# raahii/dcvgan

Measured on AMD Instinct MI355X. Metric: videos/sec per G+D step, 16x64x64 RGB+depth, higher is better.
Workload: dtype f32

## Files before the change

### dcvgan_amd/csrc/conv_mfma.hip

```cpp
#include "dcv_common.h"

#include <algorithm>
#include <cstdlib>
#include <map>
#include <mutex>
#include <string>
#include <type_traits>
#include <vector>

namespace dcv {

thread_local char g_err[512] = {0};
std::atomic<uint64_t> g_launches{0};
thread_local char g_last_kernel[160] = {0};
#define DCV_NOTE_KERNEL(...) snprintf(g_last_kernel, sizeof(g_last_kernel), __VA_ARGS__)

typedef float f32x16 __attribute__((ext_vector_type(16)));
typedef __bf16 bf16x8 __attribute__((ext_vector_type(8)));

std::atomic<int> g_precision{0};
struct BnView {
    const float* bx; const float* gamma; const float* beta; const float* mean; const float* invstd;
    int64_t bx_sn;
    int32_t bx_sc, bx_sh, cbn, act;
// ... 817 lines not shown
#else
#define DCV_STAMP_OUT()
#endif

    if (slabmode) {
        float* __restrict__ sl = a.slab + (int64_t)blockIdx.y * a.OCp * a.slab_mp;
#pragma unroll
        for (int j = 0; j < TM; ++j)
#pragma unroll
            for (int i = 0; i < TOC; ++i)
#pragma unroll
                for (int r = 0; r < 16; ++r) {
                    const int oc = oc0 + (woc * TOC + i) * 32 + (r & 3) + 8 * (r >> 2) + 4 * lhi;
                    sl[(int64_t)oc * a.slab_mp + (m0 - a.rag_m0) + (wm * TM + j) * 32 + l31] = acc[i][j][r];
                }
        DCV_STAMP_OUT()
        return;
    }
    gather_epilogue<TOC, TM>(a, acc, m0, wm * TM * 32, l31, lhi, oc0 + woc * TOC * 32, n0);
    if (a.stat) tile_bn_partials<TOC, TM, WOC, WM>(a, acc, smem, tid, lane, woc, wm, oc0, m_t);
    DCV_STAMP_OUT()
}

__global__ __launch_bounds__(256) void splitk_reduce_kernel(const GatherArgsPack pack, int S) {
    const GatherArgs& a = pack.c[blockIdx.y];
    const uint32_t Mp = (uint32_t)a.slab_mp, M = (uint32_t)a.M, q4 = Mp >> 2;
    if (q4 == 0) return;
    const uint32_t idx = blockIdx.x * 256u + threadIdx.x;
    const uint32_t oc = idx / q4, ml = (idx - oc * q4) * 4, m = ml + (uint32_t)a.rag_m0;
    if (oc >= (uint32_t)a.OC || m >= M) return;
    const float4* __restrict__ p = reinterpret_cast<const float4*>(a.slab + (int64_t)oc * Mp + ml);
    const int64_t stride = ((int64_t)a.OCp * Mp) >> 2;
    float4 v0 = {0.f, 0.f, 0.f, 0.f}, v1 = v0, v2 = v0, v3 = v0;
    int k = 0;
    for (; k + 3 < S; k += 4) {
        const float4 t0 = p[(int64_t)k * stride], t1 = p[(int64_t)(k + 1) * stride], t2 = p[(int64_t)(k + 2) * stride], t3 = p[(int64_t)(k + 3) * stride];
        v0.x += t0.x; v0.y += t0.y; v0.z += t0.z; v0.w += t0.w;
        v1.x += t1.x; v1.y += t1.y; v1.z += t1.z; v1.w += t1.w;
        v2.x += t2.x; v2.y += t2.y; v2.z += t2.z; v2.w += t2.w;
        v3.x += t3.x; v3.y += t3.y; v3.z += t3.z; v3.w += t3.w;
    }
    for (; k < S; ++k) {
        const float4 t0 = p[(int64_t)k * stride];
        v0.x += t0.x; v0.y += t0.y; v0.z += t0.z; v0.w += t0.w;
    }
    const float v[4] = {(v0.x + v1.x) + (v2.x + v3.x), (v0.y + v1.y) + (v2.y + v3.y), (v0.z + v1.z) + (v2.z + v3.z), (v0.w + v1.w) + (v2.w + v3.w)};
    const int act = a.act, accumulate = a.accumulate;
    const float slope = a.slope;
    float* __restrict__ yb = a.y + a.y_off + (int64_t)oc * a.y_sc;
#pragma unroll
    for (int e = 0; e < 4; ++e) {
        const uint32_t me = m + e;
        if (me >= M) break;
        const uint32_t n = fdiv(me, a.div_sp);
        uint32_t r0 = me - n * a.div_sp.div;
        const uint32_t od = fdiv(r0, a.div_hw);
        r0 -= od * a.div_hw.div;
        const uint32_t oh = fdiv(r0, a.div_w);
        const uint32_t ow = r0 - oh * a.div_w.div;
        float* q = yb + (int64_t)n * a.y_sn + (int64_t)od * a.y_sd + (int64_t)oh * a.y_sh + (int64_t)ow * a.y_sw;
        float x = v[e];
        if (accumulate) x += *q;
        if (a.gate) x *= a.gate[q - a.y] > 0.f ? 1.f : a.gate_slope;
        *q = apply_act(x, act, slope);
    }
}

__global__ __launch_bounds__(256) void thin_gather_kernel(const GatherArgs a) {
    __shared__ float red[3][4][64];
    const int tid = threadIdx.x, lane = tid & 63;
    const int wave = __builtin_amdgcn_readfirstlane(tid >> 6);
    const int m0 = blockIdx.x * 64;
    const uint32_t n0 = fdiv((uint32_t)m0, a.div_sp);
    const __amdgpu_buffer_rsrc_t xrs = __builtin_amdgcn_make_buffer_rsrc(
        const_cast<float*>(a.x + (int64_t)n0 * a.x_sn), 0, 0x80000000u, 0x00020000);
    const int m = m0 + lane;
    int xbase4 = 0;
    uint32_t vmask = 0;
    uint32_t n = 0, od = 0, oh = 0, ow = 0;
    if (m < a.M) {
        n = fdiv((uint32_t)m, a.div_sp);
        uint32_t r = (uint32_t)m - n * a.div_sp.div;
        od = fdiv(r, a.div_hw);
        r -= od * a.div_hw.div;
        oh = fdiv(r, a.div_w);
        ow = r - oh * a.div_w.div;
        vmask = dim_mask(a.td, (int)od, 0) | dim_mask(a.th, (int)oh, 8) | dim_mask(a.tw, (int)ow, 16);
// ... 2053 lines not shown
        else if (pt) hipLaunchKernelGGL((gather_gemm_dma_kernel<A, B, C_, D, false, true, BF_>), grid, dim3(256), 0, stream, pend); \
        else hipLaunchKernelGGL((gather_gemm_dma_kernel<A, B, C_, D, false, false, BF_>), grid, dim3(256), 0, stream, pend);        \
    }
#define DCV_LAUNCH_DMA(A, B, C_, D)                                                                                           \
    {                                                                                                                         \
        if (bfm == 2) DCV_LAUNCH_DMA1(A, B, C_, D, 2) else if (bfm == 1) DCV_LAUNCH_DMA1(A, B, C_, D, 1) else DCV_LAUNCH_DMA1(A, B, C_, D, 0) \
    }
    if (tc.bn == 128 && tc.bm == 64) DCV_LAUNCH_DMA(2, 1, 2, 2)
    else if (tc.bn == 64 && tc.bm == 128) DCV_LAUNCH_DMA(2, 1, 1, 4)
    else if (tc.bn == 128) DCV_LAUNCH_DMA(2, 2, 2, 2)
    else if (tc.bn == 64) DCV_LAUNCH_DMA(2, 2, 1, 4)
    else DCV_LAUNCH_DMA(1, 2, 1, 4)
#undef DCV_LAUNCH_DMA
#undef DCV_LAUNCH_DMA1
    DCV_NOTE_KERNEL("gather_gemm_dma_kernel<%s, %s, %s, %s> (%d x %d tile, %d class%s in one launch%s%s)",
                    tc.bn == 128 ? (tc.bm == 64 ? "2, 1, 2, 2" : "2, 2, 2, 2") : tc.bn == 64 ? (tc.bm == 128 ? "2, 1, 1, 4" : "2, 2, 1, 4") : "1, 2, 1, 4",
                    ds ? "true" : "false", pt ? "true" : "false", bfm == 2 ? "2" : bfm ? "1" : "0", tc.bn, tc.bm, n, n == 1 ? "" : "es", KS > 1 ? (pend.c[0].rag_m0 > 0 ? ", ragged split-K" : ", split-K") : "",
                    bfm == 2 ? ", f32x6: fp32 on the bf16 pipe" : bfm ? ", bf16 products" : "");
    DCV_LAUNCH_CHECK();
    if (KS > 1) {
        int64_t tot = 0;
        for (int i = 0; i < n; ++i) tot = std::max<int64_t>(tot, (int64_t)OC * (pend.c[i].slab_mp / 4));
        if (tot == 0) return DCV_OK;
        hipLaunchKernelGGL(splitk_reduce_kernel, dim3((unsigned)((tot + 255) / 256), (unsigned)n), dim3(256), 0, stream, pend, KS);
        DCV_LAUNCH_CHECK();
    }
    return DCV_OK;
}

static int structured_walk(const GatherClass& c, const dcv_dims5& xd, int RC, bool dstep, bool thin) {
    if (thin) return 0;
    if (dstep) return 2;
    const int nd = c.taps[0].n, THW = c.taps[1].n * c.taps[2].n, T = nd * THW;
    const int64_t sc4 = xd.sc * 4;
    if (T > 0 && 16 % T == 0 && RC % (16 / T) == 0 && sc4 * (16 / T) < (1ll << 30)) return 1;
    if (THW == 16 && (nd == 2 || nd == 4 || nd == 8) && c.taps[0].mul == 1 && c.taps[0].base == 0 &&
        c.taps[0].delta[nd - 1] == nd - 1 && c.o_ext[0] + nd - 1 <= c.taps[0].size && sc4 < (1ll << 30)) return 3;
    return 0;
}

static inline size_t pack_elem_bytes(int precision) { return precision == 2 ? 6 : sizeof(float); }

struct GatherOp {
    const float* x = nullptr; float* y = nullptr; const float* w = nullptr;
    dcv_dims5 xd{}, yd{};
    int RC = 0, OC = 0, KH = 1, KW = 1;
    int64_t ws_o = 0, ws_r = 0;
// ... 35 lines not shown
    const int RC = op.RC, OC = op.OC;
    const char* tag = op.tag;
    TileCfg tc = pick_gather_tile(OC);
    int nlive = 0, stat_ntm = 0, ntm_min = INT32_MAX;
    auto workgroups = [&](int bm) {
        int64_t W = 0;
        for (const GatherClass& c : op.classes)
            if (live(c)) W += ((OC + tc.bn - 1) / tc.bn) * (((int64_t)yd.n * c.o_ext[0] * c.o_ext[1] * c.o_ext[2] + bm - 1) / bm);
        return W;
    };
    for (const GatherClass& c : op.classes) nlive += live(c);
    if (tc.bn >= 64) {
        const int64_t W = workgroups(tc.bm);
        const double rounds = (double)W / 1024.0, frac = rounds - (double)(int64_t)rounds;
        bool half = (rounds > 0.4 && rounds < 1.0) || (rounds >= 1.0 && rounds < 3.0 && frac > 0.15 && frac < 0.55);
        if (tg.half_m >= 0) half = tg.half_m != 0;
        if (half && rounds >= 1.0 && tg.half_m < 0 && !tg.no_lds_dma && nlive > 0 && W / nlive >= 384 &&
            rag_plan(W, ((OC + tc.bn - 1) / tc.bn) * nlive).k > 1) half = false;
        if (half) tc.bm /= 2;
    }
    RagPlan rag{0, 1};
    if (tc.bn >= 64 && !tg.no_lds_dma) {
        rag = rag_plan(workgroups(tc.bm), ((OC + tc.bn - 1) / tc.bn) * nlive);
        if (op.stats && (int64_t)OC * yd.n * yd.d * yd.h * yd.w * 4 > (160ll << 20)) rag.k = 1;
    }
    if (op.gate && tc.bn == 4) return fail(DCV_EUNSUPPORTED, "%s: the gated epilogue is not built into the thin (OC <= 4) kernels", tag);
    if (op.gate)
        for (const GatherClass& c : op.classes)
            if (c.taps[0].n * c.taps[1].n * c.taps[2].n == 0 && c.o_ext[0] > 0 && c.o_ext[1] > 0 && c.o_ext[2] > 0)
                return fail(DCV_EUNSUPPORTED, "%s: gated epilogue with a tap-less position class", tag);
    const int OCp = (OC + tc.bn - 1) / tc.bn * tc.bn;
    P->tc = tc; P->OCp = OCp; P->cls.clear(); P->pack_need = 0;
    for (const GatherClass& c : op.classes) {
        if (!live(c)) continue;
        const int ntm = (int)(((int64_t)yd.n * c.o_ext[0] * c.o_ext[1] * c.o_ext[2] + tc.bm - 1) / tc.bm);
        stat_ntm = std::max(stat_ntm, ntm);
        ntm_min = std::min(ntm_min, ntm);
    }
    P->stat_need = (size_t)nlive * stat_ntm * OCp * 2 * sizeof(float);
    bool stat_ok = op.stats && op.act == DCV_ACT_NONE && !op.accumulate && tc.bn != 4 && P->stat_need > 0 && P->stat_need <= op.stat_bytes;
    P->stat_memset = stat_ok && ntm_min != stat_ntm;
    const bool own_pack = op.pack && op.pack->buf;
    size_t pk_off = 0, ws_off = 0;
    int stat_ci = 0;
    for (size_t ci = 0; ci < op.classes.size(); ++ci) {
        const GatherClass& c = op.classes[ci];
        if (!live(c)) continue;
// ... 53 lines not shown
        cp.fmt = dma ? o.precision : 0;
        cp.dstep = dstep; cp.T = T; cp.KS2 = KS2;
        GatherArgs& a = cp.a;
        a.M = (int)M64; a.OC = OC; a.OCp = OCp; a.KIT = KIT;
        a.OD = c.o_ext[0]; a.OH = c.o_ext[1]; a.OW = c.o_ext[2];
        a.div_sp = make_fastdiv((uint32_t)(c.o_ext[0] * c.o_ext[1] * c.o_ext[2]));
        a.div_hw = make_fastdiv((uint32_t)(c.o_ext[1] * c.o_ext[2]));
        a.div_w = make_fastdiv((uint32_t)c.o_ext[2]);
        a.td = c.taps[0]; a.th = c.taps[1]; a.tw = c.taps[2];
        {
            const int64_t per = (int64_t)c.o_ext[0] * c.o_ext[1] * c.o_ext[2];
            const int64_t span = (tc.bm / per + 2) * (xd.sn < 0 ? -xd.sn : xd.sn) + (int64_t)RC * (xd.sc < 0 ? -xd.sc : xd.sc);
            if (span >= (1ll << 29) || xd.sd > INT32_MAX / 256 || xd.sh > INT32_MAX / 256 || xd.sw > INT32_MAX / 256)
                return fail(DCV_EUNSUPPORTED, "%s: input too large for 32-bit block offsets", tag);
            const int64_t yspan = (tc.bm / per + 2) * yd.sn + (int64_t)yd.d * yd.sd + (int64_t)yd.h * yd.sh + (int64_t)yd.w * yd.sw + 8 * yd.sc;
            if (yd.sn < 0 || yd.sc < 0 || yd.sd < 0 || yd.sh < 0 || yd.sw < 0 || yspan >= (1ll << 29) || (int64_t)OCp * yd.sc >= (1ll << 30))
                return fail(DCV_EUNSUPPORTED, "%s: output too large for 32-bit block offsets", tag);
        }
        a.x_sn = xd.sn; a.x_sd = (int32_t)xd.sd; a.x_sh = (int32_t)xd.sh; a.x_sw = (int32_t)xd.sw;
        a.y_sn = yd.sn; a.y_sc = yd.sc; a.y_sd = yd.sd * c.out_mul[0]; a.y_sh = yd.sh * c.out_mul[1]; a.y_sw = yd.sw * c.out_mul[2];
        a.y_off = yd.sd * c.out_off[0] + yd.sh * c.out_off[1] + yd.sw * c.out_off[2];
        a.act = op.act; a.slope = op.slope; a.accumulate = op.accumulate; a.gate_slope = op.gate_slope;
        a.kper = kper; a.Mp = Mp; a.slab_mp = slab_mp; a.rag_m0 = rag_m0;
        cp.stat = stat_ok && KS2 == 1;
        a.stat_ntm = stat_ntm; a.stat_cls = stat_ci++;
        bool thin_struct = false;
        if (tc.bn == 4 && (T == 4 || T == 9 || T == 16) && xd.sc * 4 < (1ll << 30) && (KS2 == 1 || (kper * 16) % T == 0)) {
            thin_struct = true;
            const int nh = c.taps[1].n, nw = c.taps[2].n, THW = nh * nw;
            a.s_stepA = (int32_t)(xd.sc * 4);
            for (int t = 0; t < T; ++t) {
                const int ud = t / THW, uh = (t / nw) % nh, uw = t % nw;
                a.s_local[t] = (int32_t)(4 * (c.taps[0].delta[ud] * xd.sd + c.taps[1].delta[uh] * xd.sh + c.taps[2].delta[uw] * xd.sw));
                a.s_sel[t] = (1u << ud) | (1u << (8 + uh)) | (1u << (16 + uw));
            }
        }
        {
            const int nd = c.taps[0].n, nh = c.taps[1].n, nw = c.taps[2].n, THW = nh * nw;
            const int64_t sc4 = xd.sc * 4;
            a.structured = 0;
            if (walk == 2) {
                a.structured = 2;
                a.s_log2p = nd == 2 ? 1 : nd == 4 ? 2 : 3;
                a.s_stepA = (int32_t)(sc4 * 4);
                a.s_stepD = (int32_t)(4 * xd.sd);
                a.x_back = (int32_t)((nd - 1) * xd.sd);
                for (int r = 0; r < 16; ++r) {
// ... 35 lines not shown
            const bool contig = tap_span(c.taps[1], &dminh) && tap_span(c.taps[2], &dminw);
            const int dw1 = nw >= 2 ? c.taps[2].delta[1] - c.taps[2].delta[0] : 0;
            const bool pairs = (nw == 2 || nw == 4) && (dw1 == 1 || dw1 == -1) && (nw == 2 || c.taps[2].delta[3] - c.taps[2].delta[2] == dw1);
            const int iwmin = c.taps[2].base + dminw;
            const int IWp = IW + 8, GPR = IW / 4 + 2;
            const int l2nh = ilog2(nh), l2ow = ilog2(OW);
            const bool aligned = xd.sw == 1 && IW % 4 == 0 && xd.sh % 4 == 0 && xd.sc % 4 == 0 && xd.sd % 4 == 0 && xd.sn % 4 == 0 &&
                                 (reinterpret_cast<uintptr_t>(op.x) & 15) == 0 && (a.structured != 2 || a.x_back % 4 == 0);
            if (CH > 0 && CH * nh * nw == 16 && contig && pairs && l2nh >= 0 && l2ow >= 0 && OW <= tc.bm && aligned && iwmin >= -4 &&
                (OW - 1) * c.taps[2].mul + iwmin + nw - 1 <= IW + 3 && xd.sc * 4 * CH < (1ll << 30)) {
                const int TR = tc.bm / OW;
                const int G = CH * TR * nh * GPR;
                if (G <= 4 * tc.bm) {
                    a.patch = 1; a.p_G = G; a.p_log2nh = l2nh; a.p_log2tr = ilog2(TR); a.p_log2ow = l2ow; a.p_iwp = IWp;
                    a.p_ihmin = c.taps[1].base + dminh; a.p_iwmin4 = iwmin + 4; a.p_dw1 = dw1; a.p_sc4 = (int32_t)(xd.sc * 4);
                    a.p_gpr = make_fastdiv((uint32_t)GPR);
                    for (int r = 0; r < 16; ++r) {
                        const int t = r % (nh * nw), chr = r / (nh * nw), uh = t / nw, uw = t % nw;
                        a.s_local[r] = 4 * (chr * (TR * nh * IWp) + (c.taps[1].delta[uh] - dminh) * IWp + (c.taps[2].delta[uw] - dminw));
                    }
                }
            }
        }
        if (!dma || KS2 > 1) stat_ok = false;
        if (dma) {
            cp.kind = GK::Dma;
            cp.grid = dim3((unsigned)blocks, (unsigned)KS2);
#ifdef DCV_DEBUG_TIMING
            if (tg.debug_nostore) a.p_pad2 = 0x5701;
#endif
            P->cls.push_back(cp);
            continue;
        }
        int rows_kind = 0;
        if (tc.bn == 4 && KS2 == 1 && xd.sw == 1 && c.taps[0].mul == 1 && c.taps[1].mul == 1 && c.taps[2].mul == 1 &&
            c.o_ext[2] == c.taps[2].size && !tg.no_row64 && xd.sc * 4 < (1ll << 30) && xd.sd * 4 * 8 < (1ll << 30)) {
            const int nd = c.taps[0].n, nh = c.taps[1].n, nw = c.taps[2].n, OWc = c.o_ext[2], OHc = c.o_ext[1];
            if (nd == 1 && nh == 3 && nw == 3 && OWc == 64 && OHc % 4 == 0) rows_kind = 1;
            else if (nd == 1 && nh == 2 && nw == 2 && OWc == 32 && OHc % 8 == 0) rows_kind = 2;
            else if (nd == 4 && nh == 2 && nw == 2 && OWc == 32 && OHc % 8 == 0) rows_kind = 3;
            if (rows_kind) {
                int dminh = 0, dminw = 0;
                const bool ok = tap_span(c.taps[1], &dminh) && tap_span(c.taps[2], &dminw);
                cp.rows_iw0 = c.taps[2].base + dminw;
                if (!ok || cp.rows_iw0 < -1 || cp.rows_iw0 + nw - 1 > 1 || (rows_kind == 1 && cp.rows_iw0 != -1)) rows_kind = 0;
                else {
                    a.p_ihmin = c.taps[1].base + dminh;
// ... 41 lines not shown
                    cp.groups = OHc % 16 == 0 ? 4 : OHc % 8 == 0 ? 2 : 1;
                    cp.grid = dim3((unsigned)(M64 / 256 / cp.groups));
                    cp.kind = GK::WidenMfma;
                    if (const HeadBnRequest* hb = o.headbn) {
                        if (OCp == 128 && OC == 128 && (hb->cbn == 32 || hb->cbn == 64 || hb->cbn == 96) && !op.accumulate && op.act == DCV_ACT_NONE && c.o_ext[0] == 1 &&
                            hb->bxd.n == yd.n && hb->bxd.c == hb->cbn && hb->bxd.d == 1 && hb->bxd.h == OHc && hb->bxd.w == 64 &&
                            hb->bxd.sn >= 0 && hb->bxd.sc >= 0 && hb->bxd.sh >= 0 && hb->bxd.sw >= 0 &&
                            (int64_t)hb->cbn * hb->bxd.sc + (int64_t)OHc * hb->bxd.sh + 64 * hb->bxd.sw < (1ll << 29) &&
                            (size_t)cp.grid.x * hb->cbn * 2 * sizeof(float) <= hb->partial_bytes &&
                            hb->bdxd.sn >= 0 && hb->bdxd.sc >= 0 && hb->bdxd.sh >= 0 && hb->bdxd.sw >= 0 &&
                            (int64_t)hb->cbn * hb->bdxd.sc + (int64_t)OHc * hb->bdxd.sh + 64 * hb->bdxd.sw < (1ll << 29))
                            cp.kind = GK::HeadBn;
                    }
                }
                P->cls.push_back(cp);
                continue;
            }
        }
        cp.kind = tc.bn != 4 ? GK::Gemm : thin_struct ? GK::ThinStruct : GK::ThinGather;
        cp.grid = dim3((unsigned)blocks, (unsigned)KS2);
        P->cls.push_back(cp);
    }
    P->ws_need = ws_off;
    P->stat_parts = stat_ok ? nlive * stat_ntm : 0;
    return DCV_OK;
}

static int gather_table(const GatherOp& op, const ClassPlan& cp, DevTable* tab) {
    const GatherClass& c = op.classes[cp.ci];
    const dcv_dims5& xd = op.xd;
    std::string key = device_prefix() + op.tag;
    {
        char buf[512];
        int nn = snprintf(buf, sizeof(buf), "|g%d|%d|%d|%lld|%lld|%d|%d|%lld|%lld|%lld|%lld|", (int)cp.dstep, op.RC, op.OC, (long long)op.ws_o, (long long)op.ws_r, op.KH, op.KW,
                          (long long)xd.sc, (long long)xd.sd, (long long)xd.sh, (long long)xd.sw);
        key.append(buf, nn);
        for (int d = 0; d < 3; ++d) {
            nn = snprintf(buf, sizeof(buf), "%d:", c.taps[d].n);
            key.append(buf, nn);
            for (int u = 0; u < c.taps[d].n; ++u) {
                nn = snprintf(buf, sizeof(buf), "%d,%d;", c.taps[d].delta[u], c.tap_k[d][u]);
                key.append(buf, nn);
            }
        }
    }
    return get_table(key, [&] {
// ... 69 lines not shown
        }
        break;
    }
    default: {
        const int KS2 = cp.KS2, T = cp.T;
        DCV_NOTE_KERNEL("%s (%d x %d tile%s)", cp.kind == GK::ThinStruct ? "thin_struct_kernel" : cp.kind == GK::ThinGather ? "thin_gather_kernel" : "gather_gemm_kernel",
                        tc.bn, tc.bm, KS2 > 1 ? ", split-K" : "");
        if (cp.kind == GK::ThinStruct) {
            const int rcps = KS2 > 1 ? a.kper * 16 / T : RC;
            if (T == 4) launch_thin_struct<4>(a, OC, RC, rcps, cp.grid, stream);
            else if (T == 9) launch_thin_struct<9>(a, OC, RC, rcps, cp.grid, stream);
            else launch_thin_struct<16>(a, OC, RC, rcps, cp.grid, stream);
        } else if (cp.kind == GK::ThinGather) hipLaunchKernelGGL(thin_gather_kernel, cp.grid, dim3(256), 0, stream, a);
        else if (tc.bn == 128 && tc.bm == 64) launch_gather<2, 1, 2, 2>(a, cp.grid, stream);
        else if (tc.bn == 64 && tc.bm == 128) launch_gather<2, 1, 1, 4>(a, cp.grid, stream);
        else if (tc.bn == 128) launch_gather<2, 2, 2, 2>(a, cp.grid, stream);
        else if (tc.bn == 64) launch_gather<2, 2, 1, 4>(a, cp.grid, stream);
        else launch_gather<1, 2, 1, 4>(a, cp.grid, stream);
        DCV_LAUNCH_CHECK();
        if (KS2 == 1) return DCV_OK;
        const int64_t tot = (int64_t)OC * (a.Mp / 4);
        GatherArgsPack one;
        for (int i = 0; i < 4; ++i) one.c[i] = a;
        hipLaunchKernelGGL(splitk_reduce_kernel, dim3((unsigned)((tot + 255) / 256), 1), dim3(256), 0, stream, one, KS2);
        break;
    }
    }
    DCV_LAUNCH_CHECK();
    return DCV_OK;
}

static int run_gather(const GatherOp& op, const GatherPlan& P, const CallOpts& o, const dcv_wpack* pack, void* ws, hipStream_t stream) {
    const TileCfg& tc = P.tc;
    const bool own_pack = pack && pack->buf;
    char* const wp_base = static_cast<char*>(own_pack ? pack->buf : ws);
    const bool pk_ready = own_pack && pack->ready;
    if (P.stat_memset) DCV_HIP_CHECK(hipMemsetAsync(op.stat, 0, P.stat_need, stream));
    GatherArgsPack pend;
    PackArgs packs;
    memset(&packs, 0, sizeof(packs));
    int npack = 0, packmax = 0, npend = 0, KSpend = 1;
    dim3 pend_grid(0, 1, 1);
    auto flush_pk = [&]() {
        if (npack == 0) return (int)DCV_OK;
        const int rc = flush_packs(op.w, packs, npack, packmax, op.OC, P.OCp, op.ws_o, stream);
        npack = packmax = 0;
        return rc;
// ... 792 lines not shown
    if (pack && pack->buf) { pk2 = *pack; pk2.ready = 1; c.pack = &pk2; }
    if ((rc = run_conv(c, P, o, ws, ws_bytes, stream)) != DCV_OK) return rc;
    *fused = 1;
    return DCV_OK;
}

size_t dcv_conv_packed_bytes(const dcv_conv_geom* g, const dcv_dims5* x, const dcv_dims5* y, int which) {
    ConvPlan P;
    return (which == 0 || which == 1) && plan_sizes(g, x, y, which, false, &P) == DCV_OK ? P.gp.pack_need : 0;
}

int dcv_conv_forward(const dcv_conv_geom* g, const float* x, const dcv_dims5* xd, const float* w, float* y, const dcv_dims5* yd,
                     int act, float slope, const dcv_wpack* pack, void* ws, size_t ws_bytes, void* stream) {
    ConvCall c;
    c.g = g; c.xd = xd; c.yd = yd; c.src = x; c.w = w; c.dst = y; c.act = act; c.slope = slope; c.pack = pack;
    return conv_call(c, ws, ws_bytes, stream);
}

size_t dcv_conv_stats_bytes(const dcv_conv_geom* g, const dcv_dims5* x, const dcv_dims5* y) {
    ConvPlan P;
    return plan_sizes(g, x, y, 0, true, &P) == DCV_OK && P.op.stats ? P.gp.stat_need : 0;
}

int dcv_conv_forward_stats(const dcv_conv_geom* g, const float* x, const dcv_dims5* xd, const float* w, float* y, const dcv_dims5* yd,
                           float* stat, size_t stat_bytes, int* nparts, int* pitch, const dcv_wpack* pack, void* ws, size_t ws_bytes, void* stream) {
    if (!stat || !nparts || !pitch) return fail(DCV_EINVAL, "conv_forward_stats: null pointer");
    CallOpts o; ConvCall c; ConvPlan P;
    int rc = call_opts(g, &o, "conv");
    if (rc != DCV_OK) return rc;
    c.g = g; c.xd = xd; c.yd = yd; c.src = x; c.w = w; c.dst = y; c.pack = pack;
    c.stats = true; c.stat = stat; c.stat_bytes = stat_bytes;
    if ((rc = plan_conv(c, o, &P)) != DCV_OK) return rc;
    *pitch = P.gp.OCp;
    return run_conv(c, P, o, ws, ws_bytes, stream, nparts);
}

int dcv_conv_backward_data(const dcv_conv_geom* g, const float* dy, const dcv_dims5* dyd, const float* w, float* dx, const dcv_dims5* dxd,
                           int accumulate, const dcv_wpack* pack, void* ws, size_t ws_bytes, void* stream) {
    ConvCall c;
    c.which = 1; c.g = g; c.xd = dxd; c.yd = dyd; c.src = dy; c.w = w; c.dst = dx; c.accumulate = accumulate; c.pack = pack;
    return conv_call(c, ws, ws_bytes, stream);
}

int dcv_conv_backward_data_gated(const dcv_conv_geom* g, const float* dy, const dcv_dims5* dyd, const float* w, float* dx, const dcv_dims5* dxd,
                                 int accumulate, const float* x, const dcv_dims5* xd, int act, float slope, const dcv_wpack* pack,
                                 void* ws, size_t ws_bytes, void* stream) {
// ... 72 lines not shown
```

### dcvgan_amd/layers.py

```python
from __future__ import annotations

import torch
import torch.nn as nn

from . import ops, ops_cl

import os

_FUSE_BN_STATS = os.environ.get("DCV_NO_BN_FUSION") is None
KINK_TAP = None
PREBN_TAP = None


def _tap(y, fused):
    if KINK_TAP is not None and fused is not None and fused[0] == ops.ACT_LEAKY:
        KINK_TAP.append((y.detach() > 0).cpu())
_CONVS = (nn.Conv2d, nn.Conv3d, nn.ConvTranspose2d)
_BNS = (nn.BatchNorm2d, nn.BatchNorm3d)


def _act_of(layer):
    if isinstance(layer, nn.LeakyReLU):
        return ops.ACT_LEAKY, float(layer.negative_slope)
    if isinstance(layer, nn.ReLU):
# ... 36 lines not shown
        layer = layers[i]
        nxt = layers[i + 1] if i + 1 < n else None
        if isinstance(layer, _CONVS) and ops_cl.is_cl(x):
            fused = _act_of(nxt) if nxt is not None else None
            last = i + (2 if fused is not None else 1) >= n
            box = [] if (fused is None and isinstance(nxt, _BNS) and nxt.training and _FUSE_BN_STATS) else None
            x = ops_cl.conv(x, layer.weight, geom_of(layer), *(fused or (ops.ACT_NONE, 0.0)), out=out if last else None, grad_slot=grad_slot if i == 0 else None, bn_stats=box,
                            act_slot=act_slot if (last and fused is not None) else None)
            pending = box[0] if box else None
            if PREBN_TAP is not None and fused is None and isinstance(nxt, _BNS):
                PREBN_TAP.append(x.detach().float().abs().max())
            i += 2 if fused is not None else 1
        elif isinstance(layer, _CONVS):
            fused = _act_of(nxt) if nxt is not None else None
            if fused is not None:
                x = ops.conv(x, layer.weight, geom_of(layer), fused[0], fused[1], out=out if i + 2 >= n else None, grad_slot=grad_slot if i == 0 else None,
                             act_slot=act_slot if i + 2 >= n else None, bn_link=bn_link if i == 0 else None, gate=gate if first_conv else None)
                first_conv = False
                _tap(x, fused)
                i += 2
            else:
                box = [] if (isinstance(nxt, _BNS) and nxt.training and _FUSE_BN_STATS) else None
                x = ops.conv(x, layer.weight, geom_of(layer), out=out if i + 1 >= n else None, bn_stats=box, grad_slot=grad_slot if i == 0 else None,
                             gate=gate if first_conv else None)
                first_conv = False
                pending = box[0] if box else None
                i += 1
        elif isinstance(layer, _BNS):
            j = i + 1
            drop = None
            if j < n and isinstance(layers[j], nn.Dropout2d):
                drop = layers[j]
                j += 1
            fused = _act_of(layers[j]) if j < n else None
            if fused is not None:
                j += 1
            x = batch_norm(layer, x, rng, fused or (ops.ACT_NONE, 0.0), drop, out=out if j >= n else None, partials=pending,
                           link=bn_link if (j >= n and not ops_cl.is_cl(x)) else None)
            _tap(x, fused)
            pending = None
            i = j
        elif _act_of(layer) is not None:
            code, slope = _act_of(layer)
            x = ops_cl.act(x, code, slope) if ops_cl.is_cl(x) else ops.act(x, code, slope)
            _tap(x, (code, slope))
            i += 1
        elif hasattr(layer, "use_noise") and hasattr(layer, "sigma"):
# ... 14 lines not shown
```

### dcvgan_amd/native.py

```python
from __future__ import annotations

import ctypes as C
import os
import threading
from typing import Optional, Sequence

import torch

_HERE = os.path.dirname(os.path.abspath(__file__))
LIB_PATH = os.environ.get("DCV_LIB_PATH") or os.path.join(_HERE, "libdcvgan_hip.so")

ACT_NONE, ACT_LEAKY, ACT_TANH = 0, 1, 2
DCV_OK, DCV_EINVAL, DCV_EWORKSPACE, DCV_EHIP, DCV_EUNSUPPORTED = 0, -1, -2, -3, -4


class NativeError(RuntimeError):
    pass


class Dims5(C.Structure):
    _fields_ = [("n", C.c_int32), ("c", C.c_int32), ("d", C.c_int32), ("h", C.c_int32), ("w", C.c_int32),
                ("sn", C.c_int64), ("sc", C.c_int64), ("sd", C.c_int64), ("sh", C.c_int64), ("sw", C.c_int64)]


# ... 10 lines not shown
                ("mfma", C.c_int32)]

    def key(self):
        return tuple(getattr(self, f) for f, _ in self._fields_)


_P = C.c_void_p
_D = C.POINTER(Dims5)
_G = C.POINTER(ConvGeom)
_SIGS = {
    "dcv_last_error": (C.c_char_p, []),
    "dcv_version": (C.c_int, []),
    "dcv_abi_struct_sizes": (None, [C.POINTER(C.c_size_t)]),
    "dcv_conv_effective_precision": (C.c_int, [_G]),
    "dcv_launch_count": (C.c_uint64, []),
    "dcv_debug_kernel_info": (C.c_int, [C.c_char_p, C.c_size_t]),
    "dcv_debug_last_kernel": (C.c_char_p, []),
    "dcv_set_precision": (C.c_int, [C.c_int]),
    "dcv_get_precision": (C.c_int, []),
    "dcv_conv_workspace_bytes": (C.c_size_t, [_G, _D, _D, C.c_int]),
    "dcv_conv_packed_bytes": (C.c_size_t, [_G, _D, _D, C.c_int]),
    "dcv_conv_forward": (C.c_int, [_G, _P, _D, _P, _P, _D, C.c_int, C.c_float, _P, _P, C.c_size_t, _P]),
    "dcv_conv_stats_bytes": (C.c_size_t, [_G, _D, _D]),
    "dcv_conv_forward_stats": (C.c_int, [_G, _P, _D, _P, _P, _D, _P, C.c_size_t, C.POINTER(C.c_int), C.POINTER(C.c_int), _P, _P, C.c_size_t, _P]),
    "dcv_conv_backward_data": (C.c_int, [_G, _P, _D, _P, _P, _D, C.c_int, _P, _P, C.c_size_t, _P]),
    "dcv_conv_backward_data_gated": (C.c_int, [_G, _P, _D, _P, _P, _D, C.c_int, _P, _D, C.c_int, C.c_float, _P, _P, C.c_size_t, _P]),
    "dcv_bn_forward_stats_only": (C.c_int, [_P, _D, _P, _P, _P, _P, _P, C.c_float, C.c_float, _P, C.c_int, C.c_int, _P]),
    "dcv_bn_apply": (C.c_int, [_P, _D, _P, _D, _P, _P, _P, _P, _P, C.c_int, C.c_float, _P]),
    "dcv_conv_forward_bn": (C.c_int, [_G, _P, _D, _P, _P, _D, C.c_int, C.c_float, _P, _P, C.c_size_t, C.c_int, _P, _D, _P, _P, _P, _P, C.c_int, C.c_float, _P]),
    "dcv_conv_backward_weight_bn": (C.c_int, [_G, _P, _D, _P, _D, _P, C.c_int, _P, C.c_size_t, C.c_int, _P, _D, _P, _P, _P, _P, C.c_int, C.c_float, _P]),
    "dcv_conv_backward_data_bn_workspace_bytes": (C.c_size_t, [_D, C.c_int]),
    "dcv_conv_backward_data_bn": (C.c_int, [_G, _P, _D, _P, _P, _D, _P, _P, C.c_size_t, C.c_int, _P, _D, _P, _P, _P, _P, C.c_int, C.c_float, _P, _D, _P, _P,
                                            _P, C.c_size_t, C.POINTER(C.c_int), _P]),
    "dcv_conv_backward_weight": (C.c_int, [_G, _P, _D, _P, _D, _P, _P, C.c_size_t, _P]),
    "dcv_conv_backward_weight_acc": (C.c_int, [_G, _P, _D, _P, _D, _P, C.c_int, _P, C.c_size_t, _P]),
    "dcv_bn_workspace_bytes": (C.c_size_t, [C.c_int]),
    "dcv_bn_act_forward": (C.c_int, [_P, _D, _P, _D, _P, _P, _P, _P, _P, _P, _P, _P, C.c_int, C.c_float, C.c_float, C.c_int, C.c_float, _P, C.c_size_t, _P]),
    "dcv_bn_act_forward_stats": (C.c_int, [_P, _D, _P, _D, _P, _P, _P, _P, _P, _P, _P, _P, C.c_float, C.c_float, C.c_int, C.c_float, _P, C.c_int, C.c_int, _P, C.c_size_t, _P]),
    "dcv_bn_act_backward": (C.c_int, [_P, _D, _P, _D, _P, _D, _P, _P, _P, _P, _P, C.c_int, C.c_int, C.c_float, _P, _P, _P, C.c_size_t, _P]),
    "dcv_act_forward": (C.c_int, [_P, _D, _P, _D, C.c_int, C.c_float, _P]),
    "dcv_act_backward": (C.c_int, [_P, _D, _P, _D, _P, _D, C.c_int, C.c_float, _P]),
    "dcv_axpby": (C.c_int, [_P, _D, C.c_float, _P, _D, C.c_float, _P, _D, _P]),
    "dcv_noise_add": (C.c_int, [_P, _D, _P, _D, C.c_float, C.c_uint64, C.c_uint64, _P]),
    "dcv_normal_fill": (C.c_int, [_P, C.c_int64, C.c_uint64, C.c_uint64, _P]),
    "dcv_normal_fill_many": (C.c_int, [_P, C.c_int64, C.c_int64, C.c_uint64, C.c_uint64, _P]),
    "dcv_dropout_mask": (C.c_int, [_P, C.c_int64, C.c_float, C.c_uint64, C.c_uint64, _P]),
# ... 172 lines not shown
```

### dcvgan_amd/ops.py

```python
from __future__ import annotations

import ctypes as C
import os
from typing import Optional, Tuple

import torch
from torch.autograd import Function

from . import native as N
from .native import ACT_LEAKY, ACT_NONE, ACT_TANH, ConvGeom, check, dims5, lib, ptr, stream_ptr

__all__ = ["invalidate_packed_weights", "conv", "bn_act", "act", "noise_add", "cat_channels", "temporal_diff", "gan_loss", "gru_sequence",
           "normal", "dropout2d_mask", "conv_geom", "ACT_NONE", "ACT_LEAKY", "ACT_TANH"]


def _dense(t: torch.Tensor) -> torch.Tensor:
    if any(s == 0 and n > 1 for s, n in zip(t.stride(), t.shape)):
        return t.contiguous()
    return t


_POISON = bool(int(os.environ.get("DCV_DEBUG_POISON", "0")))


# ... 199 lines not shown


_HEAD_BN_FUSION = os.environ.get("DCV_NO_HEAD_BN_FUSION") is None


class BnLink:
    __slots__ = ("x", "gamma", "beta", "stats", "act", "slope", "task", "dx", "dgb", "stream", "defer", "deferred", "out", "_keep")

    def __init__(self, defer: bool = False):
        self.x = self.gamma = self.beta = self.stats = self.dx = self.dgb = self.out = None
        self.act, self.slope, self.task, self.stream = ACT_NONE, 0.0, -1, -1
        self.defer, self.deferred = bool(defer) and _HEAD_BN_FUSION and os.environ.get("DCV_NO_HEAD_BN_DEFER") is None, False

    def view_args(self):
        bxd = dims5(self.x)
        self._keep = bxd
        return (self.x.shape[1], ptr(self.x), C.byref(bxd), ptr(self.gamma), ptr(self.beta), ptr(self.stats[0]), ptr(self.stats[1]), self.act, self.slope)


class _Conv(Function):
    _epoch = [object()]

    @staticmethod
    def forward(ctx, x, w, g: ConvGeom, act: int, slope: float, out=None, bn_stats=None, grad_slot=None, act_slot=None, bn_link=None, gate=None):
        N._require(x, "conv input"); N._require(w, "conv weight")
        ctx.grad_slot = grad_slot
        ctx.gate = gate if (_GATED_DGRAD and gate is not None and gate[1] is not None) else None
        ctx.bn_link = bn_link if _HEAD_BN_FUSION else None
        ctx.act_slot = act_slot if (act_slot is not None and act == ACT_LEAKY) else None
        if ctx.act_slot is not None:
            ctx.act_slot.act, ctx.act_slot.act_applied = (act, slope), False
        if x.shape[1] != g.cin:
            raise N.NativeError(f"conv: input has {x.shape[1]} channels, module expects {g.cin}")
        if not w.is_contiguous():
            raise N.NativeError("conv: weights must be contiguous (torch layout)")
        y = _dest(out, _out_shape(g, x), x.device)
        xd, yd = dims5(x), dims5(y)
        L = lib()
        need = L.dcv_conv_workspace_bytes(C.byref(g), C.byref(xd), C.byref(yd), 0)
        if need == 0:
            raise N.NativeError("conv forward: " + L.dcv_last_error().decode())
        wsp, wsn = _ws("conv", need, x.device)
        ctx.pack = pc = _pack_of(w)
        pk = pc.get(w, 0, g, x, y, xd, yd) if pc is not None else None
        pkp = C.byref(pk) if pk is not None else None
        ctx.bn_deferred = False
        lk = ctx.bn_link
        if lk is not None and lk.deferred:
            rc = L.dcv_conv_forward_bn(C.byref(g), ptr(x), C.byref(xd), ptr(w), ptr(y), C.byref(yd), act, slope, pkp, wsp, wsn, *lk.view_args(), stream_ptr())
            if rc == N.DCV_EUNSUPPORTED:
                od, bxd_ = dims5(lk.out), dims5(lk.x)
                check(L.dcv_bn_apply(ptr(lk.x), C.byref(bxd_), ptr(lk.out), C.byref(od), ptr(lk.gamma), ptr(lk.beta), ptr(lk.stats[0]), ptr(lk.stats[1]), None,
                                     lk.act, lk.slope, stream_ptr()), "dcv_bn_apply")
                lk.deferred = False
            else:
                check(rc, "dcv_conv_forward_bn")
                _PackCache.commit(pk)
                ctx.bn_deferred = True
                ctx.g, ctx.act, ctx.slope = g, act, slope
                ctx.save_for_backward(x, w, y if act != ACT_NONE else None)
                return y
        sbytes = L.dcv_conv_stats_bytes(C.byref(g), C.byref(xd), C.byref(yd)) if (bn_stats is not None and act == ACT_NONE) else 0
        if sbytes:
            stat = _empty((sbytes // 4,), x.device)
            nparts, pitch = C.c_int(0), C.c_int(0)
            check(L.dcv_conv_forward_stats(C.byref(g), ptr(x), C.byref(xd), ptr(w), ptr(y), C.byref(yd), ptr(stat), sbytes,
                                           C.byref(nparts), C.byref(pitch), pkp, wsp, wsn, stream_ptr()), "dcv_conv_forward_stats")
            if nparts.value > 0:
                bn_stats.append((stat, nparts.value, pitch.value))
        else:
            check(L.dcv_conv_forward(C.byref(g), ptr(x), C.byref(xd), ptr(w), ptr(y), C.byref(yd), act, slope, pkp, wsp, wsn, stream_ptr()), "dcv_conv_forward")
        _PackCache.commit(pk)
        ctx.g, ctx.act, ctx.slope = g, act, slope
        ctx.save_for_backward(x, w, y if act != ACT_NONE else None)
        return y

    @staticmethod
    def backward(ctx, dy):
        x, w, y = ctx.saved_tensors
        g = ctx.g
        L = lib()
        dy = _dense(dy)
        fused_away = ctx.act_slot is not None and bool(ctx.act_slot.act_applied)
        if ctx.act_slot is not None:
            ctx.act_slot.act_applied = max(0, int(ctx.act_slot.act_applied) - 1)
# ... 90 lines not shown
            if ctx.bn_deferred:
                if tgt is None:
                    dw = _empty(w.shape, w.device)
                check(L.dcv_conv_backward_weight_bn(C.byref(g), ptr(x), C.byref(xd), ptr(dy), C.byref(dyd), C.c_void_p(tgt) if tgt is not None else ptr(dw),
                                                    int(tgt is not None), wsp, wsn, *ctx.bn_link.view_args(), stream_ptr()), "dcv_conv_backward_weight_bn")
                if tgt is None and _OWN_ACCUMULATION:
                    note_first(w, dw)
            elif tgt is not None:
                check(L.dcv_conv_backward_weight_acc(C.byref(g), ptr(x), C.byref(xd), ptr(dy), C.byref(dyd), C.c_void_p(tgt), 1, wsp, wsn, stream_ptr()),
                      "dcv_conv_backward_weight_acc")
            else:
                slot = getattr(w, "_dcv_grad_slot", None)
                if slot is not None and w.grad is None and getattr(w, "_dcv_slot_epoch", None) is not _Conv._epoch[0]:
                    w._dcv_slot_epoch = _Conv._epoch[0]
                    b = getattr(w, "_dcv_bucket", None)
                    if b is not None and b() is not None:
                        b().before_slot_write(w)
                    dw = slot.detach()
                else:
                    dw = _empty(w.shape, w.device)
                check(L.dcv_conv_backward_weight(C.byref(g), ptr(x), C.byref(xd), ptr(dy), C.byref(dyd), ptr(dw), wsp, wsn, stream_ptr()), "dcv_conv_backward_weight")
                if _OWN_ACCUMULATION:
                    note_first(w, dw)
        return dx, dw, None, None, None, None, None, None, None, None, None


def new_backward_epoch():
    _Conv._epoch[0] = object()


def conv(x, w, g: ConvGeom, act: int = ACT_NONE, slope: float = 0.0, out=None, bn_stats=None, grad_slot=None, act_slot=None, bn_link=None, gate=None):
    return _Conv.apply(x, w, g, act, float(slope), None if out is None else _Out(out), bn_stats, grad_slot, act_slot, bn_link, gate)


class _BnAct(Function):
    @staticmethod
    def forward(ctx, x, gamma, beta, running_mean, running_var, mask, training: bool, momentum: float, eps: float, act: int, slope: float, out=None,
                partials=None, nbt=None, link=None):
        N._require(x, "bn input")
        ctx.link = link
        L = lib()
        Cn = x.shape[1]
        y = _dest(out, x.shape, x.device)
        stats = _empty((2, Cn), x.device)
        xd, yd = dims5(x), dims5(y)
        wsp, wsn = _ws("bn", L.dcv_bn_workspace_bytes(Cn), x.device)
        if link is not None:
            link.deferred = False
        if link is not None and link.defer and partials is not None and training and mask is None and act in (ACT_NONE, ACT_LEAKY) and x.dim() == 4 and x.is_contiguous() \
                and x.shape[3] == 64 and x.shape[1] % 32 == 0:
            stat, nparts, pitch = partials.v
            check(L.dcv_bn_forward_stats_only(ptr(x), C.byref(xd), ptr(running_mean), ptr(running_var), ptr(nbt), ptr(stats[0]), ptr(stats[1]), momentum, eps,
                                              ptr(stat), nparts, pitch, stream_ptr()), "dcv_bn_forward_stats_only")
            link.deferred, link.out = True, y.detach()
        elif partials is not None and training:
# ... 419 lines not shown
```

### include/dcvgan_hip.h

```cpp
#ifndef DCVGAN_HIP_H
#define DCVGAN_HIP_H

#include <stddef.h>
#include <stdint.h>

#ifdef __cplusplus
extern "C" {
#endif

#define DCV_OK 0
#define DCV_EINVAL (-1)
#define DCV_EWORKSPACE (-2)
#define DCV_EHIP (-3)
#define DCV_EUNSUPPORTED (-4)

#define DCV_ACT_NONE 0
#define DCV_ACT_LEAKY 1
#define DCV_ACT_TANH 2

typedef struct dcv_dims5 {
    int32_t n, c, d, h, w;
    int64_t sn, sc, sd, sh, sw;
} dcv_dims5;

// ... 8 lines not shown

const char* dcv_last_error(void);
int dcv_version(void);
void dcv_abi_struct_sizes(size_t out[3]);
uint64_t dcv_launch_count(void);
int dcv_set_precision(int mode);
int dcv_get_precision(void);
int dcv_conv_effective_precision(const dcv_conv_geom* g);
const char* dcv_debug_last_kernel(void);
int dcv_debug_kernel_info(char* buf, size_t n);

size_t dcv_conv_workspace_bytes(const dcv_conv_geom* g, const dcv_dims5* x, const dcv_dims5* y, int which );
typedef struct dcv_wpack {
    float* buf;
    size_t bytes;
    int32_t ready;
    int32_t precision;
} dcv_wpack;
size_t dcv_conv_packed_bytes(const dcv_conv_geom* g, const dcv_dims5* x, const dcv_dims5* y, int which );
int dcv_conv_forward(const dcv_conv_geom* g, const float* x, const dcv_dims5* xd, const float* w,
                     float* y, const dcv_dims5* yd, int act, float slope, const dcv_wpack* pack,
                     void* ws, size_t ws_bytes, void* stream);
size_t dcv_conv_stats_bytes(const dcv_conv_geom* g, const dcv_dims5* x, const dcv_dims5* y);
int dcv_conv_forward_stats(const dcv_conv_geom* g, const float* x, const dcv_dims5* xd, const float* w, float* y, const dcv_dims5* yd,
                           float* stat, size_t stat_bytes, int* nparts, int* pitch, const dcv_wpack* pack, void* ws, size_t ws_bytes, void* stream);
int dcv_conv_backward_data(const dcv_conv_geom* g, const float* dy, const dcv_dims5* dyd, const float* w,
                           float* dx, const dcv_dims5* dxd, int accumulate, const dcv_wpack* pack,
                           void* ws, size_t ws_bytes, void* stream);
int dcv_conv_backward_data_gated(const dcv_conv_geom* g, const float* dy, const dcv_dims5* dyd, const float* w,
                                 float* dx, const dcv_dims5* dxd, int accumulate,
                                 const float* x, const dcv_dims5* xd, int act, float slope, const dcv_wpack* pack,
                                 void* ws, size_t ws_bytes, void* stream);
int dcv_bn_forward_stats_only(const float* x, const dcv_dims5* xd, float* running_mean, float* running_var, int64_t* num_batches_tracked, float* save_mean, float* save_invstd,
                              float momentum, float eps, const float* stat, int nparts, int pitch, void* stream);
int dcv_bn_apply(const float* x, const dcv_dims5* xd, float* y, const dcv_dims5* yd, const float* gamma, const float* beta, const float* save_mean, const float* save_invstd,
                 const float* mask, int act, float slope, void* stream);
int dcv_conv_forward_bn(const dcv_conv_geom* g, const float* x, const dcv_dims5* xd, const float* w, float* y, const dcv_dims5* yd, int act, float slope,
                        const dcv_wpack* pack, void* ws, size_t ws_bytes, int cbn, const float* bn_x, const dcv_dims5* bn_xd, const float* gamma, const float* beta,
                        const float* save_mean, const float* save_invstd, int bn_act, float bn_slope, void* stream);
int dcv_conv_backward_weight_bn(const dcv_conv_geom* g, const float* x, const dcv_dims5* xd, const float* dy, const dcv_dims5* dyd, float* dw, int accumulate,
                                void* ws, size_t ws_bytes, int cbn, const float* bn_x, const dcv_dims5* bn_xd, const float* gamma, const float* beta,
                                const float* save_mean, const float* save_invstd, int bn_act, float bn_slope, void* stream);
size_t dcv_conv_backward_data_bn_workspace_bytes(const dcv_dims5* dxd, int cbn);
int dcv_conv_backward_data_bn(const dcv_conv_geom* g, const float* dy, const dcv_dims5* dyd, const float* w, float* dx, const dcv_dims5* dxd, const dcv_wpack* pack,
                              void* ws, size_t ws_bytes, int cbn, const float* bn_x, const dcv_dims5* bn_xd, const float* gamma, const float* beta,
                              const float* save_mean, const float* save_invstd, int act, float slope, float* bn_dx, const dcv_dims5* bn_dxd, float* dgamma, float* dbeta,
// ... 140 lines not shown
```

Measured before the change: 658.6.

## Fuse BatchNorm statistics into split-K reduce epilogue for conv forward

The split-K reduce kernel gains a templated STAT mode that accumulates per-channel sum and sum of squares over its output tile and writes BN partials. Split-K convolutions therefore no longer lose fused BN statistics. The heuristic that forced split-K off for large stat-producing convs is also removed, so those layers keep split-K parallelism. A new API reports split count, and the generator path opts in via split_stats. This saves a separate BN statistics pass over the activations, at the cost of a shuffle reduction and partial writes in the reduce kernel.

```diff
diff --git a/dcvgan_amd/csrc/conv_mfma.hip b/dcvgan_amd/csrc/conv_mfma.hip
--- a/dcvgan_amd/csrc/conv_mfma.hip
+++ b/dcvgan_amd/csrc/conv_mfma.hip
@@ -863,13 +863,17 @@
     DCV_STAMP_OUT()
 }
 
-__global__ __launch_bounds__(256) void splitk_reduce_kernel(const GatherArgsPack pack, int S) {
+template <bool STAT>
+__global__ __launch_bounds__(256) void splitk_reduce_kernel(const GatherArgsPack pack, int S, int g4) {
     const GatherArgs& a = pack.c[blockIdx.y];
     const uint32_t Mp = (uint32_t)a.slab_mp, M = (uint32_t)a.M, q4 = Mp >> 2;
     if (q4 == 0) return;
     const uint32_t idx = blockIdx.x * 256u + threadIdx.x;
     const uint32_t oc = idx / q4, ml = (idx - oc * q4) * 4, m = ml + (uint32_t)a.rag_m0;
-    if (oc >= (uint32_t)a.OC || m >= M) return;
+    const bool mine = oc < (uint32_t)a.OC && m < M;
+    if (!STAT && !mine) return;
+    float s1 = 0.f, s2 = 0.f;
+    if (mine) {
     const float4* __restrict__ p = reinterpret_cast<const float4*>(a.slab + (int64_t)oc * Mp + ml);
     const int64_t stride = ((int64_t)a.OCp * Mp) >> 2;
     float4 v0 = {0.f, 0.f, 0.f, 0.f}, v1 = v0, v2 = v0, v3 = v0;
@@ -903,7 +907,18 @@
         float x = v[e];
         if (accumulate) x += *q;
         if (a.gate) x *= a.gate[q - a.y] > 0.f ? 1.f : a.gate_slope;
-        *q = apply_act(x, act, slope);
+        x = apply_act(x, act, slope);
+        *q = x;
+        if constexpr (STAT) { s1 += x; s2 += x * x; }
+    }
+    }
+    if constexpr (STAT) {
+        for (int off = 1; off < g4; off <<= 1) { s1 += __shfl_xor(s1, off); s2 += __shfl_xor(s2, off); }
+        if (oc < (uint32_t)a.OC && (idx & (uint32_t)(g4 - 1)) == 0) {
+            const uint32_t m_t = m / (4u * (uint32_t)g4);
+            float2* __restrict__ dst = reinterpret_cast<float2*>(a.stat + ((int64_t)(a.stat_cls * a.stat_ntm + (int)m_t) * a.OCp + oc) * 2);
+            *dst = make_float2(s1, s2);
+        }
     }
 }
 
@@ -3003,7 +3018,8 @@
         int64_t tot = 0;
         for (int i = 0; i < n; ++i) tot = std::max<int64_t>(tot, (int64_t)OC * (pend.c[i].slab_mp / 4));
         if (tot == 0) return DCV_OK;
-        hipLaunchKernelGGL(splitk_reduce_kernel, dim3((unsigned)((tot + 255) / 256), (unsigned)n), dim3(256), 0, stream, pend, KS);
+        if (pend.c[0].stat) hipLaunchKernelGGL(splitk_reduce_kernel<true>, dim3((unsigned)((tot + 255) / 256), (unsigned)n), dim3(256), 0, stream, pend, KS, tc.bm / 4);
+        else hipLaunchKernelGGL(splitk_reduce_kernel<false>, dim3((unsigned)((tot + 255) / 256), (unsigned)n), dim3(256), 0, stream, pend, KS, tc.bm / 4);
         DCV_LAUNCH_CHECK();
     }
     return DCV_OK;
@@ -3085,7 +3101,6 @@
     RagPlan rag{0, 1};
     if (tc.bn >= 64 && !tg.no_lds_dma) {
         rag = rag_plan(workgroups(tc.bm), ((OC + tc.bn - 1) / tc.bn) * nlive);
-        if (op.stats && (int64_t)OC * yd.n * yd.d * yd.h * yd.w * 4 > (160ll << 20)) rag.k = 1;
     }
     if (op.gate && tc.bn == 4) return fail(DCV_EUNSUPPORTED, "%s: the gated epilogue is not built into the thin (OC <= 4) kernels", tag);
     if (op.gate)
@@ -3185,7 +3200,7 @@
         a.y_off = yd.sd * c.out_off[0] + yd.sh * c.out_off[1] + yd.sw * c.out_off[2];
         a.act = op.act; a.slope = op.slope; a.accumulate = op.accumulate; a.gate_slope = op.gate_slope;
         a.kper = kper; a.Mp = Mp; a.slab_mp = slab_mp; a.rag_m0 = rag_m0;
-        cp.stat = stat_ok && KS2 == 1;
+        cp.stat = stat_ok && dma;
         a.stat_ntm = stat_ntm; a.stat_cls = stat_ci++;
         bool thin_struct = false;
         if (tc.bn == 4 && (T == 4 || T == 9 || T == 16) && xd.sc * 4 < (1ll << 30) && (KS2 == 1 || (kper * 16) % T == 0)) {
@@ -3267,7 +3282,7 @@
                 }
             }
         }
-        if (!dma || KS2 > 1) stat_ok = false;
+        if (!dma) stat_ok = false;
         if (dma) {
             cp.kind = GK::Dma;
             cp.grid = dim3((unsigned)blocks, (unsigned)KS2);
@@ -3355,6 +3370,8 @@
         P->cls.push_back(cp);
     }
     P->ws_need = ws_off;
+    if (!stat_ok)
+        for (ClassPlan& cp : P->cls) cp.stat = false;
     P->stat_parts = stat_ok ? nlive * stat_ntm : 0;
     return DCV_OK;
 }
@@ -3470,7 +3487,7 @@
         const int64_t tot = (int64_t)OC * (a.Mp / 4);
         GatherArgsPack one;
         for (int i = 0; i < 4; ++i) one.c[i] = a;
-        hipLaunchKernelGGL(splitk_reduce_kernel, dim3((unsigned)((tot + 255) / 256), 1), dim3(256), 0, stream, one, KS2);
+        hipLaunchKernelGGL(splitk_reduce_kernel<false>, dim3((unsigned)((tot + 255) / 256), 1), dim3(256), 0, stream, one, KS2, tc.bm / 4);
         break;
     }
     }
@@ -4309,6 +4326,14 @@
     return plan_sizes(g, x, y, 0, true, &P) == DCV_OK && P.op.stats ? P.gp.stat_need : 0;
 }
 
+int dcv_conv_split_parts(const dcv_conv_geom* g, const dcv_dims5* x, const dcv_dims5* y, int which) {
+    ConvPlan P;
+    if ((which != 0 && which != 1) || plan_sizes(g, x, y, which, false, &P) != DCV_OK) return 0;
+    int k = 1;
+    for (const ClassPlan& cp : P.gp.cls) k = std::max(k, cp.KS2);
+    return k;
+}
+
 int dcv_conv_forward_stats(const dcv_conv_geom* g, const float* x, const dcv_dims5* xd, const float* w, float* y, const dcv_dims5* yd,
                            float* stat, size_t stat_bytes, int* nparts, int* pitch, const dcv_wpack* pack, void* ws, size_t ws_bytes, void* stream) {
     if (!stat || !nparts || !pitch) return fail(DCV_EINVAL, "conv_forward_stats: null pointer");
diff --git a/dcvgan_amd/layers.py b/dcvgan_amd/layers.py
--- a/dcvgan_amd/layers.py
+++ b/dcvgan_amd/layers.py
@@ -82,7 +82,7 @@
             else:
                 box = [] if (isinstance(nxt, _BNS) and nxt.training and _FUSE_BN_STATS) else None
                 x = ops.conv(x, layer.weight, geom_of(layer), out=out if i + 1 >= n else None, bn_stats=box, grad_slot=grad_slot if i == 0 else None,
-                             gate=gate if first_conv else None)
+                             gate=gate if first_conv else None, split_stats=True)
                 first_conv = False
                 pending = box[0] if box else None
                 i += 1
diff --git a/dcvgan_amd/native.py b/dcvgan_amd/native.py
--- a/dcvgan_amd/native.py
+++ b/dcvgan_amd/native.py
@@ -56,6 +56,7 @@
     "dcv_conv_packed_bytes": (C.c_size_t, [_G, _D, _D, C.c_int]),
     "dcv_conv_forward": (C.c_int, [_G, _P, _D, _P, _P, _D, C.c_int, C.c_float, _P, _P, C.c_size_t, _P]),
     "dcv_conv_stats_bytes": (C.c_size_t, [_G, _D, _D]),
+    "dcv_conv_split_parts": (C.c_int, [_G, _D, _D, C.c_int]),
     "dcv_conv_forward_stats": (C.c_int, [_G, _P, _D, _P, _P, _D, _P, C.c_size_t, C.POINTER(C.c_int), C.POINTER(C.c_int), _P, _P, C.c_size_t, _P]),
     "dcv_conv_backward_data": (C.c_int, [_G, _P, _D, _P, _P, _D, C.c_int, _P, _P, C.c_size_t, _P]),
     "dcv_conv_backward_data_gated": (C.c_int, [_G, _P, _D, _P, _P, _D, C.c_int, _P, _D, C.c_int, C.c_float, _P, _P, C.c_size_t, _P]),
diff --git a/dcvgan_amd/ops.py b/dcvgan_amd/ops.py
--- a/dcvgan_amd/ops.py
+++ b/dcvgan_amd/ops.py
@@ -245,7 +245,7 @@
     _epoch = [object()]
 
     @staticmethod
-    def forward(ctx, x, w, g: ConvGeom, act: int, slope: float, out=None, bn_stats=None, grad_slot=None, act_slot=None, bn_link=None, gate=None):
+    def forward(ctx, x, w, g: ConvGeom, act: int, slope: float, out=None, bn_stats=None, grad_slot=None, act_slot=None, bn_link=None, gate=None, split_stats=False):
         N._require(x, "conv input"); N._require(w, "conv weight")
         ctx.grad_slot = grad_slot
         ctx.gate = gate if (_GATED_DGRAD and gate is not None and gate[1] is not None) else None
@@ -284,6 +284,8 @@
                 ctx.save_for_backward(x, w, y if act != ACT_NONE else None)
                 return y
         sbytes = L.dcv_conv_stats_bytes(C.byref(g), C.byref(xd), C.byref(yd)) if (bn_stats is not None and act == ACT_NONE) else 0
+        if sbytes and not split_stats and L.dcv_conv_split_parts(C.byref(g), C.byref(xd), C.byref(yd), 0) != 1:
+            sbytes = 0
         if sbytes:
             stat = _empty((sbytes // 4,), x.device)
             nparts, pitch = C.c_int(0), C.c_int(0)
@@ -420,15 +422,15 @@
                 check(L.dcv_conv_backward_weight(C.byref(g), ptr(x), C.byref(xd), ptr(dy), C.byref(dyd), ptr(dw), wsp, wsn, stream_ptr()), "dcv_conv_backward_weight")
                 if _OWN_ACCUMULATION:
                     note_first(w, dw)
-        return dx, dw, None, None, None, None, None, None, None, None, None
+        return dx, dw, None, None, None, None, None, None, None, None, None, None
 
 
 def new_backward_epoch():
     _Conv._epoch[0] = object()
 
 
-def conv(x, w, g: ConvGeom, act: int = ACT_NONE, slope: float = 0.0, out=None, bn_stats=None, grad_slot=None, act_slot=None, bn_link=None, gate=None):
-    return _Conv.apply(x, w, g, act, float(slope), None if out is None else _Out(out), bn_stats, grad_slot, act_slot, bn_link, gate)
+def conv(x, w, g: ConvGeom, act: int = ACT_NONE, slope: float = 0.0, out=None, bn_stats=None, grad_slot=None, act_slot=None, bn_link=None, gate=None, split_stats: bool = False):
+    return _Conv.apply(x, w, g, act, float(slope), None if out is None else _Out(out), bn_stats, grad_slot, act_slot, bn_link, gate, bool(split_stats))
 
 
 class _BnAct(Function):
diff --git a/include/dcvgan_hip.h b/include/dcvgan_hip.h
--- a/include/dcvgan_hip.h
+++ b/include/dcvgan_hip.h
@@ -54,6 +54,7 @@
                      float* y, const dcv_dims5* yd, int act, float slope, const dcv_wpack* pack,
                      void* ws, size_t ws_bytes, void* stream);
 size_t dcv_conv_stats_bytes(const dcv_conv_geom* g, const dcv_dims5* x, const dcv_dims5* y);
+int dcv_conv_split_parts(const dcv_conv_geom* g, const dcv_dims5* x, const dcv_dims5* y, int which);
 int dcv_conv_forward_stats(const dcv_conv_geom* g, const float* x, const dcv_dims5* xd, const float* w, float* y, const dcv_dims5* yd,
                            float* stat, size_t stat_bytes, int* nparts, int* pitch, const dcv_wpack* pack, void* ws, size_t ws_bytes, void* stream);
 int dcv_conv_backward_data(const dcv_conv_geom* g, const float* dy, const dcv_dims5* dyd, const float* w,
```

Measured after the change: 657.9. No clear change (-0.1%).
